# facebookresearch/vsc2022

Measured on AMD Instinct MI355X. Metric: query-videos localized/sec @ 512-d SSCD, higher is better.
Workload: dtype fp32 results; int8 / fp16 MFMA pre-filters; 1 GPU; BASELINE configs[3]: full pipeline incl. score normalisation + TN localisation, 40000 query videos split over 1 GPU(s), 2000000 reference + 2000000 noise frames; query_videos_per_gpu=40000, query_frames_per_gpu=1000000, ref_frames=2000000, dim=512, global_k=48000000, candidates=1000000, pairs_localized=200000, matches=446939, hits=48000000, score_normalisation_in_step=True, parallelism=single GPU

## Files before the change

### vsc2022_amd/csrc/tn.hip

```cpp
#include <cfloat>

#include "kernels.h"

namespace vscmi {

typedef float f32x16 __attribute__((ext_vector_type(16)));
typedef float f32x4 __attribute__((ext_vector_type(4)));


template <class IDX>
struct TnStateT {
    int lq, lr, top, ms, n_nodes, sink, sink_q, sink_r;
    unsigned top_magic;
    float min_sim;
    const IDX* tidx;
    const float* tsim;
    const IDX* ilo;
    const IDX* ihi;
};

template <class IDX>
__device__ __forceinline__ int tn_div_top(const TnStateT<IDX>& g, int x) {
    return g.top == 1 ? x : (int)__umulhi((unsigned)x, g.top_magic);
}
template <class IDX>
__device__ __forceinline__ int tn_node_q(const TnStateT<IDX>& g, int v) { return v == 0 ? -1 : tn_div_top(g, v - 1); }
template <class IDX>
__device__ __forceinline__ int tn_node_k(const TnStateT<IDX>& g, int v) { return (v - 1) - tn_div_top(g, v - 1) * g.top; }
template <class IDX>
__device__ __forceinline__ int tn_node_r(const TnStateT<IDX>& g, int v) { return v == 0 ? -1 : g.tidx[v - 1]; }

template <class IDX>
__device__ __forceinline__ bool tn_edge_ok(const TnStateT<IDX>& g, int qi, int a, int d, int b) {
    const int qj = qi + d;
    const int ra = g.tidx[qi * g.top + a], rb = g.tidx[qj * g.top + b];
    const int rd = rb - ra;
    if (!(rd > 0 && rd < g.ms)) return false;
    const int lo = g.ilo[qi * g.ms + d], hi = g.ihi[qi * g.ms + d];
    if (lo <= hi && !(hi < ra || lo > rb)) return false;
    return g.tsim[qj * g.top + b] >= g.min_sim;
}

template <class IDX>
__device__ __forceinline__ bool tn_sink_ok(const TnStateT<IDX>& g, int u) {
    if (u == g.sink) return false;
    const int qu = tn_node_q(g, u), ru = tn_node_r(g, u);
    return g.sink_q > qu && g.sink_r > ru && g.sink_q - qu <= g.ms && g.sink_r - ru <= g.ms;
}

template <class IDX>
__device__ __forceinline__ int tn_edge_bit(const TnStateT<IDX>& g, int qi, int a, int d, int b) {
    return (((qi + d) * g.top + b) * g.ms + d) * g.top + a;
}

__device__ __forceinline__ unsigned long long first_max_key(float v, int o) {
    const float vz = v + 0.0f;
    const unsigned b = __float_as_uint(vz);
    unsigned hi = (b & 0x80000000u) ? ~b : (b | 0x80000000u);
    hi = (vz != vz) ? 1u : hi;
    const unsigned long long k = ((unsigned long long)hi << 32) | (unsigned)(0x7fffffff - o);
    return o < 0 ? 0ull : k;
}
__device__ __forceinline__ void first_max_unkey(unsigned long long k, float& v, int& o) {
    const unsigned hi = (unsigned)(k >> 32);
    const float kv = __uint_as_float((hi & 0x80000000u) ? (hi & 0x7fffffffu) : ~hi);
    v = k ? kv : 0.0f;
    o = k ? 0x7fffffff - (int)(unsigned)k : -1;
}
template <int FIRST_OFF>
__device__ __forceinline__ void first_max_reduce(float& v, int& o) {
    unsigned long long k = first_max_key(v, o);
#pragma unroll
    for (int off = FIRST_OFF; off >= 1; off >>= 1) {
        const unsigned long long ok = __shfl_xor(k, off);
        k = ok > k ? ok : k;
    }
    first_max_unkey(k, v, o);
}
__device__ __forceinline__ void wave_first_max(float& v, int& o) { first_max_reduce<32>(v, o); }
__device__ __forceinline__ void half_first_max(float& v, int& o) { first_max_reduce<16>(v, o); }


#ifdef VSC_TN_PROFILE
__device__ unsigned long long tn_prof[8];
#define TN_T0() unsigned long long t_prof = __builtin_readcyclecounter()
#define TN_T(k)                                                                          \
    do {                                                                                 \
        const unsigned long long t_now = __builtin_readcyclecounter();                   \
        if (threadIdx.x == 0) atomicAdd(&tn_prof[k], t_now - t_prof);                    \
        t_prof = t_now;                                                                  \
    } while (0)
#else
#define TN_T0() do {} while (0)
#define TN_T(k) do {} while (0)
#endif

template <class IDX, bool GSTATE>
__global__ __launch_bounds__(64) void tn_pair_kernel(TnPairArgs a) {
    extern __shared__ __attribute__((aligned(16))) char smem_lds[];
    char* const smem = GSTATE ? a.state + (int64_t)blockIdx.x * a.state_bytes : smem_lds;
    const int lane = threadIdx.x;
    if ((int)blockIdx.x >= a.n_work) return;
    const int pidx = a.work[blockIdx.x];
    int64_t qrow0 = 0, rrow0 = 0;
    int lq, lr;
    if (a.sims_in) {
        lq = a.sims_lq[pidx];
        lr = a.sims_lr[pidx];
    } else {
        const int qv = a.pair_q[pidx], rv = a.pair_r[pidx];
        qrow0 = a.q_off[qv];
        rrow0 = a.r_off[rv];
        lq = (int)(a.q_off[qv + 1] - qrow0);
        lr = (int)(a.r_off[rv + 1] - rrow0);
    }
    const int ms = a.prm.tn_max_step > 1 ? a.prm.tn_max_step : 1;
    const int top_cap = a.prm.tn_top_k;
    const int top = top_cap < lr ? top_cap : lr;
    int32_t* o_nbox = a.out_nbox + pidx;
    int32_t* o_boxes = a.out_boxes + (int64_t)pidx * VSC_TN_MAX_BOXES * 4;
    float* o_bmax = a.out_boxmax + (int64_t)pidx * VSC_TN_MAX_BOXES;
    if (lq <= 0 || top <= 0) {
        if (lane == 0) *o_nbox = 0;
        return;
    }
    const int n_nodes = 1 + lq * top;

    size_t off = 0;
    IDX* tidx = reinterpret_cast<IDX*>(smem + off);
    off += (size_t)a.max_lq * top_cap * sizeof(IDX);
    off = (off + 15) & ~(size_t)15;
    float* tsim = reinterpret_cast<float*>(smem + off);
    off += (size_t)a.max_lq * top_cap * 4;
    IDX* ilo = reinterpret_cast<IDX*>(smem + off);
    off += (size_t)a.max_lq * ms * sizeof(IDX);
    IDX* ihi = reinterpret_cast<IDX*>(smem + off);
    off += (size_t)a.max_lq * ms * sizeof(IDX);
    off = (off + 15) & ~(size_t)15;
    unsigned int* zero = reinterpret_cast<unsigned int*>(smem + off);
    const int zero_words = (lq * top * ms * top + 31) / 32;
    off += ((size_t)a.max_lq * top_cap * ms * top_cap + 31) / 32 * 4;
    off = (off + 15) & ~(size_t)15;
    float* dist = reinterpret_cast<float*>(smem + off);
    off += (size_t)(1 + a.max_lq * top_cap) * 4;
    IDX* par = reinterpret_cast<IDX*>(smem + off);
    off += (size_t)(1 + a.max_lq * top_cap) * sizeof(IDX);
    IDX* order = reinterpret_cast<IDX*>(smem + off);
    off += (size_t)(1 + a.max_lq * top_cap) * sizeof(IDX);
    IDX* indeg = reinterpret_cast<IDX*>(smem + off);
    off += (size_t)(1 + a.max_lq * top_cap) * sizeof(IDX);
    off = (off + 15) & ~(size_t)15;
    int* boxes = reinterpret_cast<int*>(smem + off);
    off += (size_t)VSC_TN_MAX_BOXES * 16;
    unsigned long long* okmask = reinterpret_cast<unsigned long long*>(smem + off);
    off += (size_t)a.max_lq * ((top_cap + 1) / 2) * 8;
    off = (off + 63) & ~(size_t)63;
    float* sims;
    if (a.sims_in) sims = const_cast<float*>(a.sims_in) + a.sims_off[pidx];
    else if ((int64_t)lq * lr <= a.lds_tile_floats) sims = reinterpret_cast<float*>(smem + off);
    else sims = a.slab + (int64_t)blockIdx.x * a.slab_floats;

    TN_T0();
    if (!a.sims_in) {
        const int hi = lane >> 5, l31 = lane & 31;
        const int nkg = a.dpad / 8;
        for (int qb = 0; qb < lq; qb += 32)
            for (int rb = 0; rb < lr; rb += 64) {
                const bool two = rb + 32 < lr;
                const float* ap = a.qfeat + (qrow0 + qb + l31) * a.dpad + hi * 4;
                const float* bp0 = a.rfeat + (rrow0 + rb + l31) * a.dpad + hi * 4;
                const float* bp1 = bp0 + (two ? 32 * (int64_t)a.dpad : 0);
                f32x16 acc0, acc1;
#pragma unroll
                for (int r = 0; r < 16; ++r) acc0[r] = acc1[r] = 0.0f;
                if (two) {
#pragma unroll 4
                    for (int g = 0; g < nkg; ++g) {
                        const f32x4 av = *reinterpret_cast<const f32x4*>(ap + g * 8);
                        const f32x4 bv0 = *reinterpret_cast<const f32x4*>(bp0 + g * 8);
                        const f32x4 bv1 = *reinterpret_cast<const f32x4*>(bp1 + g * 8);
#pragma unroll
                        for (int s = 0; s < 4; ++s) {
                            acc0 = __builtin_amdgcn_mfma_f32_32x32x2f32(av[s], bv0[s], acc0, 0, 0, 0);
                            acc1 = __builtin_amdgcn_mfma_f32_32x32x2f32(av[s], bv1[s], acc1, 0, 0, 0);
                        }
                    }
                } else {
#pragma unroll 4
                    for (int g = 0; g < nkg; ++g) {
                        const f32x4 av = *reinterpret_cast<const f32x4*>(ap + g * 8);
                        const f32x4 bv = *reinterpret_cast<const f32x4*>(bp0 + g * 8);
#pragma unroll
                        for (int s = 0; s < 4; ++s)
                            acc0 = __builtin_amdgcn_mfma_f32_32x32x2f32(av[s], bv[s], acc0, 0, 0, 0);
                    }
                }
#pragma unroll
                for (int r = 0; r < 16; ++r) {
                    const int q = qb + (r & 3) + 8 * (r >> 2) + 4 * hi;
                    const int rr = rb + l31;
                    if (q < lq && rr < lr) sims[(int64_t)q * lr + rr] = acc0[r] + a.bias;
                    if (two && q < lq && rr + 32 < lr) sims[(int64_t)q * lr + rr + 32] = acc1[r] + a.bias;
                }
            }
    }
    for (int x = lane; x < zero_words; x += 64) zero[x] = 0;
    __threadfence_block();
    __syncthreads();
    TN_T(0);

    if (top_cap <= 8 && (lq >= 16 || lr <= 128)) {
        for (int q0 = 0; q0 < lq; q0 += 64) {
            const int q = q0 + lane;
            float ts[8];
            int ti[8];
#pragma unroll
            for (int e = 0; e < 8; ++e) {
                ts[e] = -INFINITY;
                ti[e] = -1;
            }
            if (q < lq) {
                const float* row = sims + (int64_t)q * lr;
                for (int r = 0; r < lr; ++r) {
                    const float sv = row[r];
                    if (!(sv > ts[7]) && ti[7] >= 0) continue;
#pragma unroll
                    for (int e = 7; e >= 1; --e) {
                        const bool empty_above = ti[e - 1] < 0;
                        const bool up = empty_above || sv > ts[e - 1];
                        const bool here = !up && (ti[e] < 0 || sv > ts[e]);
                        ts[e] = up ? ts[e - 1] : (here ? sv : ts[e]);
                        ti[e] = up ? ti[e - 1] : (here ? r : ti[e]);
                    }
                    if (ti[0] < 0 || sv > ts[0]) {
                        ts[0] = sv;
                        ti[0] = r;
                    }
                }
#pragma unroll
                for (int e = 0; e < 8; ++e)
                    if (e < top) {
                        tidx[q * top + e] = (IDX)ti[e];
                        tsim[q * top + e] = ts[e];
                    }
            }
        }
    } else {
        for (int q = 0; q < lq; ++q) {
            const float* row = sims + (int64_t)q * lr;
            float prev_s = INFINITY;
            int prev_r = -1;
            for (int e = 0; e < top; ++e) {
                float bs = 0.0f;
                int br = -1;
                for (int r = lane; r < lr; r += 64) {
                    const float s = row[r];
                    const bool after = (s < prev_s) || (s == prev_s && r > prev_r);
                    if (after && (br < 0 || s > bs)) {
                        bs = s;
                        br = r;
                    }
                }
                wave_first_max(bs, br);
                if (lane == 0) {
                    tidx[q * top + e] = (IDX)br;
                    tsim[q * top + e] = bs;
                }
                prev_s = bs;
                prev_r = br;
            }
        }
    }
    __syncthreads();

    TnStateT<IDX> g;
    g.lq = lq; g.lr = lr; g.top = top; g.ms = ms; g.n_nodes = n_nodes; g.sink = n_nodes - 1;
    g.sink_q = lq - 1;
    g.sink_r = tidx[(lq - 1) * top + top - 1];
    g.min_sim = a.prm.min_sim;
    g.top_magic = (unsigned)((0x100000000ull + (unsigned)top - 1u) / (unsigned)top);
    g.tidx = tidx; g.tsim = tsim; g.ilo = ilo; g.ihi = ihi;

    for (int qi = lane; qi < lq; qi += 64) {
        int lo = 1, hi = 0;
        for (int d = 1; d < ms; ++d) {
            ilo[qi * ms + d] = (IDX)lo;
            ihi[qi * ms + d] = (IDX)hi;
            if (qi + d >= lq) continue;
            int nlo = lo, nhi = hi;
            for (int b = 0; b < top; ++b) {
                bool any = false;
                for (int aa = 0; aa < top && !any; ++aa) any = tn_edge_ok(g, qi, aa, d, b);
                if (any) {
                    const int rb = tidx[(qi + d) * top + b];
                    if (nlo > nhi) nlo = nhi = rb;
                    else {
                        nlo = rb < nlo ? rb : nlo;
                        nhi = rb > nhi ? rb : nhi;
                    }
                }
            }
            lo = nlo;
            hi = nhi;
        }
    }
    __syncthreads();

    TN_T(1);
    const int P = (ms - 1) * top;
    int nbox = 0;
    bool have_order = false;
    const int hw_half = lane >> 5, hw_o = lane & 31;
    const int hw_d = ms - 1 - hw_o / top, hw_aa = hw_o % top;
    const int hw_bit_off = hw_d * top + hw_aa + hw_half * ms * top;
    const int hw_pred_off = 1 + hw_aa - hw_d * top;
    for (int it = 0; it <= a.prm.max_path; ++it) {
        if (lane == 0) {
            dist[0] = 0.0f;
            par[0] = 0;
        }
        __syncthreads();
        for (int qj = 0; qj < lq; ++qj) {
            int b_first = 0;
            if (P <= 32) {
                const int half = hw_half, o = hw_o, d = hw_d, aa = hw_aa;
                const int qi = qj - d;
                const int pred = qj * top + hw_pred_off;
                for (int b0 = 0; b0 < top; b0 += 2) {
                    const int b = b0 + half;
                    const int v = 1 + qj * top + b;
                    const bool mine = b < top && v != g.sink;
                    float c = 0.0f;
                    int oo = -1;
                    const int mslot = qj * ((top + 1) / 2) + (b0 >> 1);
                    bool ok;
                    if (it == 0) {
                        ok = mine && o < P && qi >= 0 && tn_edge_ok(g, qi, aa, d, b);
                        const unsigned long long m = __ballot(ok);
                        if (lane == 0) okmask[mslot] = m;
                    } else {
                        ok = (okmask[mslot] >> lane) & 1ull;
                    }
                    if (ok) {
                        const int bit = (qj * top + b0) * ms * top + hw_bit_off;
                        const bool z = (zero[bit >> 5] >> (bit & 31)) & 1u;
                        const float w = z ? 0.0f : tsim[qj * top + b];
                        c = dist[pred] + w;
                        oo = o;
                    }
                    half_first_max(c, oo);
                    const int pw = __shfl(pred, (lane & 32) | (oo < 0 ? 0 : oo));
                    if (mine && o == 0) {
                        if (oo < 0 || !(c >= 0.0f)) {
                            dist[v] = 0.0f;
                            par[v] = (IDX)v;
                        } else {
                            dist[v] = c;
                            par[v] = (IDX)pw;
                        }
                    }
                }
                b_first = (qj == lq - 1) ? top - 1 : top;
            }
            if (qj == lq - 1) TN_T(2);
            for (int b = b_first; b < top; ++b) {
                const int v = 1 + qj * top + b;
                const bool is_sink = (v == g.sink);
                float best = 0.0f;
                int arg = -1;
                for (int o0 = 0; o0 < P; o0 += 64) {
                    const int o = o0 + lane;
                    float c = 0.0f;
                    int oo = -1;
                    if (o < P) {
                        const int d = ms - 1 - o / top, aa = o % top;
                        const int qi = qj - d;
                        if (qi >= 0 && tn_edge_ok(g, qi, aa, d, b)) {
                            const int bit = tn_edge_bit(g, qi, aa, d, b);
                            const bool z = (zero[bit >> 5] >> (bit & 31)) & 1u;
                            const float w = (z || is_sink) ? 0.0f : tsim[qj * top + b];
                            c = dist[1 + qi * top + aa] + w;
                            oo = o;
                        }
                    }
                    wave_first_max(c, oo);
                    if (oo >= 0 && (arg < 0 || c > best)) {
                        best = c;
                        arg = oo;
                    }
                }
                int arg_node = -1;
                if (arg >= 0) arg_node = 1 + (qj - (ms - 1 - arg / top)) * top + arg % top;
                if (is_sink) {
                    for (int u0 = 0; u0 < n_nodes - 1; u0 += 64) {
                        const int u = u0 + lane;
                        float c = 0.0f;
                        int oo = -1;
                        if (u < n_nodes - 1 && tn_sink_ok(g, u)) {
                            bool regular = false;
                            if (u != 0) {
                                const int qi = tn_node_q(g, u), aa = tn_node_k(g, u);
                                const int d = qj - qi;
                                if (d >= 1 && d < ms) regular = tn_edge_ok(g, qi, aa, d, b);
                            }
                            if (!regular) {
                                c = dist[u] + 0.0f;
                                oo = u;
                            }
                        }
                        wave_first_max(c, oo);
                        if (oo >= 0 && (arg_node < 0 || c > best)) {
                            best = c;
                            arg_node = oo;
                        }
                    }
                }
                if (lane == 0) {
                    if (arg_node < 0 || !(best >= 0.0f)) {
                        dist[v] = 0.0f;
                        par[v] = (IDX)v;
                    } else {
                        dist[v] = best;
                        par[v] = (IDX)arg_node;
                    }
                }
            }
            __syncthreads();
        }

        TN_T(3);
        float mx = -FLT_MAX;
        int mxn = -1;
        for (int v = lane; v < n_nodes; v += 64) {
            const float dv = dist[v];
            if (mxn < 0 || dv > mx) {
                mx = dv;
                mxn = v;
            }
        }
        wave_first_max(mx, mxn);
        int ties = 0;
        for (int v = lane; v < n_nodes; v += 64) ties += (dist[v] == mx) ? 1 : 0;
#pragma unroll
        for (int off2 = 32; off2 >= 1; off2 >>= 1) ties += __shfl_xor(ties, off2);
        int vend = mxn;
        if (!(mx > 0.0f)) {
            vend = 0;
        } else if (ties > 1) {
            if (!have_order) {
                for (int v = lane; v < n_nodes; v += 64) {
                    int deg = 0;
                    if (v != 0) {
                        const int qj = tn_node_q(g, v), b = tn_node_k(g, v);
                        for (int d = 1; d < ms; ++d) {
                            const int qi = qj - d;
                            if (qi < 0) break;
                            for (int aa = 0; aa < top; ++aa) deg += tn_edge_ok(g, qi, aa, d, b) ? 1 : 0;
                        }
                        if (v == g.sink) {
                            for (int u = 0; u < n_nodes - 1; ++u) {
                                if (!tn_sink_ok(g, u)) continue;
                                bool regular = false;
                                if (u != 0) {
                                    const int qi = tn_node_q(g, u), aa = tn_node_k(g, u);
                                    const int d = qj - qi;
                                    if (d >= 1 && d < ms) regular = tn_edge_ok(g, qi, aa, d, b);
                                }
                                deg += regular ? 0 : 1;
                            }
                        }
                    }
                    indeg[v] = (IDX)deg;
                }
                __syncthreads();
                if (lane == 0) {
                    int head = 0, tail = 0;
                    for (int v = 0; v < n_nodes; ++v)
                        if (indeg[v] == 0) order[tail++] = (IDX)v;
                    while (head < tail) {
                        const int u = order[head++];
                        bool to_sink_regular = false;
                        if (u != 0) {
                            const int qi = tn_node_q(g, u), aa = tn_node_k(g, u);
                            for (int d = 1; d < ms && qi + d < lq; ++d)
                                for (int b = 0; b < top; ++b)
                                    if (tn_edge_ok(g, qi, aa, d, b)) {
                                        const int v = 1 + (qi + d) * top + b;
                                        if (v == g.sink) to_sink_regular = true;
                                        if (--indeg[v] == 0) order[tail++] = (IDX)v;
                                    }
                        }
                        if (!to_sink_regular && tn_sink_ok(g, u))
                            if (--indeg[g.sink] == 0) order[tail++] = (IDX)g.sink;
                    }
                }
                have_order = true;
                __syncthreads();
            }
            int bestpos = 0x7fffffff;
            for (int t = lane; t < n_nodes; t += 64)
                if (dist[order[t]] == mx && t < bestpos) bestpos = t;
#pragma unroll
            for (int off2 = 32; off2 >= 1; off2 >>= 1) {
                const int o2 = __shfl_xor(bestpos, off2);
                bestpos = o2 < bestpos ? o2 : bestpos;
            }
            vend = order[bestpos];
        }

        TN_T(4);
        int accepted = 0, stop = 0;
        int bq0 = 0, br0 = 0, bq1 = 0, br1 = 0;
        if (lane == 0) {
            int cnt = 0;
            for (int v = vend;;) {
                const int u = par[v];
                if (v != 0 && v != g.sink) ++cnt;
                if (u == v) break;
                if (u != 0) {
                    const int qi = tn_node_q(g, u), aa = tn_node_k(g, u);
                    const int qj = tn_node_q(g, v), b = tn_node_k(g, v);
                    const int d = qj - qi;
                    if (d >= 1 && d < ms && tn_edge_ok(g, qi, aa, d, b)) {
                        const int bit = tn_edge_bit(g, qi, aa, d, b);
                        zero[bit >> 5] |= 1u << (bit & 31);
                    }
                }
                v = u;
            }
            if (cnt == 0) {
                stop = 1;
            } else {
                int plen = 0;
                for (int v = vend;;) {
                    indeg[plen++] = (IDX)v;
                    if (par[v] == v) break;
                    v = par[v];
                }
                float score = 0.0f;
                int qmin = 0, qmax = 0, rmin = 0, rmax = 0, c2 = 0;
                for (int x = plen - 1; x >= 0; --x) {
                    const int v = indeg[x];
                    if (v == 0 || v == g.sink) continue;
                    const int q = tn_node_q(g, v), r = tn_node_r(g, v);
                    score += tsim[v - 1];
                    if (c2 == 0) {
                        qmin = qmax = q;
                        rmin = rmax = r;
                    } else {
                        qmin = q < qmin ? q : qmin;
                        qmax = q > qmax ? q : qmax;
                        rmin = r < rmin ? r : rmin;
                        rmax = r > rmax ? r : rmax;
                    }
                    ++c2;
                }
                if (!(score > 0.0f)) qmin = qmax = rmin = rmax = 0;
                const int dq = qmax - qmin, dr = rmax - rmin;
                const float ave = __fdiv_rn((float)(dr + dq), 2.0f);
                bool ok = (ave != 0.0f) && (__fdiv_rn(score, ave) > a.prm.min_sim) &&
                          ((dr < dq ? dr : dq) > a.prm.min_length);
                if (ok && nbox > 0) {
                    float mxi = -INFINITY;
                    for (int kx = 0; kx < nbox; ++kx) {
                        const int* o = boxes + 4 * kx;
                        const float lt0 = (float)(qmin > o[0] ? qmin : o[0]);
                        const float lt1 = (float)(rmin > o[1] ? rmin : o[1]);
                        const float rb0 = (float)(qmax < o[2] ? qmax : o[2]);
                        const float rb1 = (float)(rmax < o[3] ? rmax : o[3]);
                        const float w = rb0 - lt0 > 0.0f ? rb0 - lt0 : 0.0f;
                        const float h = rb1 - lt1 > 0.0f ? rb1 - lt1 : 0.0f;
                        const float inter = __fmul_rn(w, h);
                        const float aa2 = __fmul_rn((float)dq, (float)dr);
                        const float ab = __fmul_rn((float)(o[2] - o[0]), (float)(o[3] - o[1]));
                        const float iou = __fdiv_rn(inter, __fsub_rn(__fadd_rn(aa2, ab), inter));
                        mxi = iou > mxi ? iou : mxi;
                    }
                    ok = mxi < a.prm.max_iou;
                }
                if (ok && nbox < VSC_TN_MAX_BOXES) {
                    boxes[4 * nbox + 0] = qmin;
                    boxes[4 * nbox + 1] = rmin;
                    boxes[4 * nbox + 2] = qmax;
                    boxes[4 * nbox + 3] = rmax;
                    accepted = 1;
                    bq0 = qmin; br0 = rmin; bq1 = qmax; br1 = rmax;
                }
            }
        }
        stop = __shfl(stop, 0);
        accepted = __shfl(accepted, 0);
        __syncthreads();
        TN_T(5);
        if (stop) break;
        if (accepted) {
            bq0 = __shfl(bq0, 0); br0 = __shfl(br0, 0); bq1 = __shfl(bq1, 0); br1 = __shfl(br1, 0);
            float m = -INFINITY;
            const int w = br1 - br0, h = bq1 - bq0;
            for (int y = 0; y < h; ++y) {
                const float* srow = sims + (int64_t)(bq0 + y) * lr + br0;
                for (int x = lane; x < w; x += 64) {
                    const float s = srow[x];
                    m = s > m ? s : m;
                }
            }
#pragma unroll
            for (int off2 = 32; off2 >= 1; off2 >>= 1) {
                const float o2 = __shfl_xor(m, off2);
                m = o2 > m ? o2 : m;
            }
            if (lane == 0) {
                o_boxes[4 * nbox + 0] = bq0;
                o_boxes[4 * nbox + 1] = br0;
                o_boxes[4 * nbox + 2] = bq1;
                o_boxes[4 * nbox + 3] = br1;
                o_bmax[nbox] = __fsub_rn(m, a.bias);
            }
            ++nbox;
        }
        TN_T(6);
    }
    if (lane == 0) *o_nbox = nbox;
}

#ifdef VSC_TN_PROFILE
extern "C" int vsc_tn_prof_read(unsigned long long* out8, int reset) {
    if (hipMemcpyFromSymbol(out8, HIP_SYMBOL(tn_prof), sizeof(tn_prof)) != hipSuccess) return -1;
    if (reset) {
        unsigned long long z[8] = {};
        if (hipMemcpyToSymbol(HIP_SYMBOL(tn_prof), z, sizeof(z)) != hipSuccess) return -1;
    }
    return 0;
}
#endif

size_t tn_state_bytes_host(int max_lq, int top_cap, int ms, int idx_bytes) {
    const size_t n_nodes = 1 + (size_t)max_lq * top_cap;
    const size_t ib = (size_t)idx_bytes;
    size_t b = 0;
    b += (size_t)max_lq * top_cap * ib;
    b = (b + 15) & ~(size_t)15;
    b += (size_t)max_lq * top_cap * 4;
    b += (size_t)max_lq * ms * ib * 2;
    b = (b + 15) & ~(size_t)15;
    b += ((size_t)max_lq * top_cap * ms * top_cap + 31) / 32 * 4;
    b = (b + 15) & ~(size_t)15;
    b += n_nodes * 4;
    b += n_nodes * ib * 3;
    b = (b + 15) & ~(size_t)15;
    b += (size_t)VSC_TN_MAX_BOXES * 16;
    b += (size_t)max_lq * ((top_cap + 1) / 2) * 8;
    b = (b + 63) & ~(size_t)63;
    return b;
}

int launch_tn_pairs(const TnPairArgs& a, size_t lds_bytes, hipStream_t stream) {
    if (a.n_work <= 0) return VSC_OK;
    static PerDeviceOnce once;
    if (a.state) {
        hipLaunchKernelGGL((tn_pair_kernel<int, true>), dim3((unsigned)a.n_work), dim3(64), 0, stream, a);
        VSC_HIP(hipGetLastError());
        return VSC_OK;
    }
    if (once.first()) {
        VSC_HIP(hipFuncSetAttribute(reinterpret_cast<const void*>(&tn_pair_kernel<short, false>),
                                    hipFuncAttributeMaxDynamicSharedMemorySize, 158 * 1024));
        once.commit();
    }
    hipLaunchKernelGGL((tn_pair_kernel<short, false>), dim3((unsigned)a.n_work), dim3(64), lds_bytes, stream, a);
    VSC_HIP(hipGetLastError());
    return VSC_OK;
}


__global__ __launch_bounds__(64) void tn_sims_kernel(TnSimsArgs a) {
    const int lane = threadIdx.x, hi = lane >> 5, l31 = lane & 31;
    const int qb = blockIdx.y * 32, rb = blockIdx.x * 32;
    const float* ap = a.qfeat + (a.qrow0 + qb + l31) * a.dpad + hi * 4;
    const float* bp = a.rfeat + (a.rrow0 + rb + l31) * a.dpad + hi * 4;
    f32x16 acc;
#pragma unroll
    for (int r = 0; r < 16; ++r) acc[r] = 0.0f;
    const int nkg = a.dpad / 8;
#pragma unroll 4
    for (int g = 0; g < nkg; ++g) {
        const f32x4 av = *reinterpret_cast<const f32x4*>(ap + g * 8);
        const f32x4 bv = *reinterpret_cast<const f32x4*>(bp + g * 8);
#pragma unroll
        for (int s = 0; s < 4; ++s) acc = __builtin_amdgcn_mfma_f32_32x32x2f32(av[s], bv[s], acc, 0, 0, 0);
    }
#pragma unroll
    for (int r = 0; r < 16; ++r) {
        const int q = qb + (r & 3) + 8 * (r >> 2) + 4 * hi;
        const int rr = rb + l31;
        if (q < a.lq && rr < a.lr) a.out[(int64_t)q * a.lr + rr] = acc[r] + a.bias;
    }
}

int launch_tn_sims(const TnSimsArgs& a, hipStream_t stream) {
    if (a.lq <= 0 || a.lr <= 0) return VSC_OK;
    hipLaunchKernelGGL(tn_sims_kernel, dim3((a.lr + 31) / 32, (a.lq + 31) / 32), dim3(64), 0, stream, a);
    VSC_HIP(hipGetLastError());
    return VSC_OK;
}

}
```

Measured before the change: 19750 query-videos/s.

## Process a whole TN graph row per wave with DPP group-of-8 max reduction

Adds a ROWPASS variant of the temporal-network longest-path kernel. Each group of 8 lanes owns one target node b and loops over up to 8 predecessor slots, replacing the half-wave-per-pair loop with a single pass per query row. Per-row edge validity is cached as one byte per lane, and the argmax is taken with packed 64-bit keys reduced by DPP lane permutes instead of wave-wide shuffles. The variant is on by default when top_k is at most 8 and the state fits in LDS, and node ids are limited to 15 bits.

```diff
diff --git a/vsc2022_amd/csrc/tn.hip b/vsc2022_amd/csrc/tn.hip
--- a/vsc2022_amd/csrc/tn.hip
+++ b/vsc2022_amd/csrc/tn.hip
@@ -1,4 +1,5 @@
 #include <cfloat>
+#include <cstdlib>
 
 #include "kernels.h"
 
@@ -79,6 +80,26 @@
 }
 __device__ __forceinline__ void wave_first_max(float& v, int& o) { first_max_reduce<32>(v, o); }
 __device__ __forceinline__ void half_first_max(float& v, int& o) { first_max_reduce<16>(v, o); }
+
+__device__ __forceinline__ unsigned first_max_hi(float v) {
+    const unsigned b = __float_as_uint(v);
+    const unsigned hi = b ^ ((unsigned)((int)b >> 31) | 0x80000000u);
+    return (v != v) ? 1u : hi;
+}
+template <int CTRL>
+__device__ __forceinline__ unsigned long long dpp_max_u64(unsigned long long k) {
+    const unsigned lo = (unsigned)k, hi = (unsigned)(k >> 32);
+    const unsigned olo = (unsigned)__builtin_amdgcn_update_dpp((int)lo, (int)lo, CTRL, 0xf, 0xf, false);
+    const unsigned ohi = (unsigned)__builtin_amdgcn_update_dpp((int)hi, (int)hi, CTRL, 0xf, 0xf, false);
+    const unsigned long long ok = ((unsigned long long)ohi << 32) | olo;
+    return ok > k ? ok : k;
+}
+__device__ __forceinline__ unsigned long long group8_max_u64(unsigned long long k) {
+    k = dpp_max_u64<0x141>(k);
+    k = dpp_max_u64<0x1b>(k);
+    k = dpp_max_u64<0xb1>(k);
+    return k;
+}
 
 
 #ifdef VSC_TN_PROFILE
@@ -95,8 +116,9 @@
 #define TN_T(k) do {} while (0)
 #endif
 
-template <class IDX, bool GSTATE>
+template <class IDX, bool GSTATE, bool ROWPASS>
 __global__ __launch_bounds__(64) void tn_pair_kernel(TnPairArgs a) {
+    static_assert(!ROWPASS || (!GSTATE && sizeof(IDX) == 2), "the row pass keeps node ids in 15 bits of its keys");
     extern __shared__ __attribute__((aligned(16))) char smem_lds[];
     char* const smem = GSTATE ? a.state + (int64_t)blockIdx.x * a.state_bytes : smem_lds;
     const int lane = threadIdx.x;
@@ -153,7 +175,8 @@
     int* boxes = reinterpret_cast<int*>(smem + off);
     off += (size_t)VSC_TN_MAX_BOXES * 16;
     unsigned long long* okmask = reinterpret_cast<unsigned long long*>(smem + off);
-    off += (size_t)a.max_lq * ((top_cap + 1) / 2) * 8;
+    unsigned char* okrow = reinterpret_cast<unsigned char*>(smem + off);
+    off += ROWPASS ? (size_t)a.max_lq * 64 : (size_t)a.max_lq * ((top_cap + 1) / 2) * 8;
     off = (off + 63) & ~(size_t)63;
     float* sims;
     if (a.sims_in) sims = const_cast<float*>(a.sims_in) + a.sims_off[pidx];
@@ -314,6 +337,20 @@
     const int hw_d = ms - 1 - hw_o / top, hw_aa = hw_o % top;
     const int hw_bit_off = hw_d * top + hw_aa + hw_half * ms * top;
     const int hw_pred_off = 1 + hw_aa - hw_d * top;
+    const int rp_b = lane >> 3, rp_T = (P + 7) >> 3;
+    int rp_da[8], rp_bit_off[8];
+    unsigned rp_klo[8];
+    if (ROWPASS) {
+#pragma unroll
+        for (int t = 0; t < 8; ++t) {
+            const int o = (lane & 7) + 8 * t;
+            const bool slot = o < P;
+            const int d = slot ? ms - 1 - o / top : 0, aa = slot ? o % top : 0;
+            rp_da[t] = slot ? (d << 4) | aa : -1;
+            rp_bit_off[t] = d * top + aa + rp_b * ms * top;
+            rp_klo[t] = ((unsigned)(63 - o) << 16) + (unsigned)(1 + aa - d * top);
+        }
+    }
     for (int it = 0; it <= a.prm.max_path; ++it) {
         if (lane == 0) {
             dist[0] = 0.0f;
@@ -322,7 +359,52 @@
         __syncthreads();
         for (int qj = 0; qj < lq; ++qj) {
             int b_first = 0;
-            if (P <= 32) {
+            if (ROWPASS) {
+                const int b = rp_b;
+                const int v = 1 + qj * top + b;
+                const bool mine = b < top && v != g.sink;
+                const int row_node = qj * top, row_bit = qj * top * ms * top;
+                unsigned okb = 0;
+                if (it == 0) {
+#pragma unroll
+                    for (int t = 0; t < 8; ++t) {
+                        if (t >= rp_T) break;
+                        const int da = rp_da[t], d = da >> 4, aa = da & 15;
+                        const bool ok = mine && da >= 0 && qj - d >= 0 && tn_edge_ok(g, qj - d, aa, d, b);
+                        okb |= ok ? 1u << t : 0u;
+                    }
+                    okrow[qj * 64 + lane] = (unsigned char)okb;
+                } else {
+                    okb = okrow[qj * 64 + lane];
+                }
+                const float wv = mine ? tsim[row_node + b] : 0.0f;
+                unsigned long long k = 0ull;
+#pragma unroll
+                for (int t = 0; t < 8; ++t) {
+                    if (t >= rp_T) break;
+                    const unsigned klo = rp_klo[t] + (unsigned)row_node;
+                    const int pred = (short)klo;
+                    const int bit = row_bit + rp_bit_off[t];
+                    const bool z = (zero[bit >> 5] >> (bit & 31)) & 1u;
+                    const float c = dist[pred < 0 ? 0 : pred] + (z ? 0.0f : wv);
+                    const unsigned hi = first_max_hi(c) & (unsigned)((int)(okb << (31 - t)) >> 31);
+                    const unsigned long long kt = ((unsigned long long)hi << 32) | klo;
+                    k = kt > k ? kt : k;
+                }
+                k = group8_max_u64(k);
+                if (mine && (lane & 7) == 0) {
+                    const unsigned hi = (unsigned)(k >> 32);
+                    const float c = __uint_as_float((hi & 0x80000000u) ? (hi & 0x7fffffffu) : ~hi);
+                    if (hi == 0u || !(c >= 0.0f)) {
+                        dist[v] = 0.0f;
+                        par[v] = (IDX)v;
+                    } else {
+                        dist[v] = c;
+                        par[v] = (IDX)((unsigned)k & 0x7fffu);
+                    }
+                }
+                b_first = (qj == lq - 1) ? top - 1 : top;
+            } else if (P <= 32) {
                 const int half = hw_half, o = hw_o, d = hw_d, aa = hw_aa;
                 const int qi = qj - d;
                 const int pred = qj * top + hw_pred_off;
@@ -634,7 +716,28 @@
 }
 #endif
 
+static bool tn_rowpass_enabled() {
+    static int on = -1;
+    if (on < 0) {
+        const char* e = getenv("VSC_TN_ROWPASS");
+        on = (e && atoi(e) == 0) ? 0 : 1;
+    }
+    return on == 1;
+}
+
+static size_t tn_state_bytes_for(int max_lq, int top_cap, int ms, int idx_bytes, bool rowpass);
+
+static bool tn_use_rowpass(int max_lq, int top_cap, int ms, int idx_bytes) {
+    if (!tn_rowpass_enabled() || idx_bytes != 2 || top_cap < 1 || top_cap > 8 || (ms - 1) * top_cap > 64) return false;
+    const size_t room = max_lq <= 256 ? (size_t)158 * 1024 - (size_t)24576 * 4 : (size_t)150 * 1024;
+    return tn_state_bytes_for(max_lq, top_cap, ms, idx_bytes, true) <= room;
+}
+
 size_t tn_state_bytes_host(int max_lq, int top_cap, int ms, int idx_bytes) {
+    return tn_state_bytes_for(max_lq, top_cap, ms, idx_bytes, tn_use_rowpass(max_lq, top_cap, ms, idx_bytes));
+}
+
+static size_t tn_state_bytes_for(int max_lq, int top_cap, int ms, int idx_bytes, bool rowpass) {
     const size_t n_nodes = 1 + (size_t)max_lq * top_cap;
     const size_t ib = (size_t)idx_bytes;
     size_t b = 0;
@@ -649,7 +752,7 @@
     b += n_nodes * ib * 3;
     b = (b + 15) & ~(size_t)15;
     b += (size_t)VSC_TN_MAX_BOXES * 16;
-    b += (size_t)max_lq * ((top_cap + 1) / 2) * 8;
+    b += rowpass ? (size_t)max_lq * 64 : (size_t)max_lq * ((top_cap + 1) / 2) * 8;
     b = (b + 63) & ~(size_t)63;
     return b;
 }
@@ -658,16 +761,22 @@
     if (a.n_work <= 0) return VSC_OK;
     static PerDeviceOnce once;
     if (a.state) {
-        hipLaunchKernelGGL((tn_pair_kernel<int, true>), dim3((unsigned)a.n_work), dim3(64), 0, stream, a);
+        hipLaunchKernelGGL((tn_pair_kernel<int, true, false>), dim3((unsigned)a.n_work), dim3(64), 0, stream, a);
         VSC_HIP(hipGetLastError());
         return VSC_OK;
     }
     if (once.first()) {
-        VSC_HIP(hipFuncSetAttribute(reinterpret_cast<const void*>(&tn_pair_kernel<short, false>),
+        VSC_HIP(hipFuncSetAttribute(reinterpret_cast<const void*>(&tn_pair_kernel<short, false, false>),
+                                    hipFuncAttributeMaxDynamicSharedMemorySize, 158 * 1024));
+        VSC_HIP(hipFuncSetAttribute(reinterpret_cast<const void*>(&tn_pair_kernel<short, false, true>),
                                     hipFuncAttributeMaxDynamicSharedMemorySize, 158 * 1024));
         once.commit();
     }
-    hipLaunchKernelGGL((tn_pair_kernel<short, false>), dim3((unsigned)a.n_work), dim3(64), lds_bytes, stream, a);
+    const int ms = a.prm.tn_max_step > 1 ? a.prm.tn_max_step : 1;
+    if (tn_use_rowpass(a.max_lq, a.prm.tn_top_k, ms, 2))
+        hipLaunchKernelGGL((tn_pair_kernel<short, false, true>), dim3((unsigned)a.n_work), dim3(64), lds_bytes, stream, a);
+    else
+        hipLaunchKernelGGL((tn_pair_kernel<short, false, false>), dim3((unsigned)a.n_work), dim3(64), lds_bytes, stream, a);
     VSC_HIP(hipGetLastError());
     return VSC_OK;
 }
```

Result: no change. 19890 query-videos/s, median of 6 (+0.7%).
